# jeffchy/RE2NN-SEQ

Hardware: AMD Instinct MI355X
Metric: tagged tokens/sec @ batch=256, seqlen=64; achieved HBM GB/s vs peak (higher is better)
Workload: dtype f32; 1 GPU; ATIS-BIO-sized onehot i-FST (--method onehot --independent 2): V=950 S=71 C=128, batch 256 x seqlen 64 per GPU, lengths U[5,64]; batches_rotated=4, parallelism=batch-sharded x1 (weights replicated)

## Files before the change

### re2nn-seq_amd/csrc/chain_regs.hip.h

```cpp
#pragma once
#include "common.hip.h"
#include "score_params.hip.h"
#include "launch_order.hip.h"
#include "chain_regs_params.hip.h"
#include "beside.hip.h"

#ifndef FARNN_ABLATE
#define FARNN_ABLATE 0
#endif

namespace farnn {

__device__ __forceinline__ void lds_flag_set(int *f, int v) {
    asm volatile("" ::: "memory");
    __hip_atomic_store(f, v, __ATOMIC_RELAXED, __HIP_MEMORY_SCOPE_WORKGROUP);
}
__device__ __forceinline__ int lds_flag_get(const int *f) {
    const int v = __hip_atomic_load(f, __ATOMIC_RELAXED, __HIP_MEMORY_SCOPE_WORKGROUP);
    asm volatile("" ::: "memory");
    return v;
}
template <int PSTR = RG_PART_STRIDE>
__device__ __forceinline__ int regs_flag_newest(const float *fbase, int lane) {
    const int *f = reinterpret_cast<const int *>(fbase) + 4 * (lane < RG_NWC ? lane : 0);
    const int v0 = lds_flag_get(f), v1 = lds_flag_get(f + PSTR);
    return max(v0, v1);
}
template <int PSTR = RG_PART_STRIDE>
__device__ __forceinline__ bool regs_rows_reached(const float *fbase, int lane, int rows) {
    return __ballot(regs_flag_newest<PSTR>(fbase, lane) < rows + 1) == 0ull;
}
template <int PSTR = RG_PART_STRIDE>
__device__ __forceinline__ int regs_rows_done(const float *fbase, int lane) {
    int v = regs_flag_newest<PSTR>(fbase, lane);
#pragma unroll
    for (int off = 1; off < 8; off <<= 1) v = min(v, __shfl_xor(v, off, WAVE));
    return __builtin_amdgcn_readfirstlane(v) - 1;
}

__device__ __forceinline__ float quad_sum(float x) {
    x += __int_as_float(__builtin_amdgcn_update_dpp(0, __float_as_int(x), 0xB1, 0xf, 0xf, true));
    x += __int_as_float(__builtin_amdgcn_update_dpp(0, __float_as_int(x), 0x4E, 0xf, 0xf, true));
    return x;
}
__device__ __forceinline__ float quad_max(float x) {
    x = fmaxf(x, __int_as_float(__builtin_amdgcn_update_dpp(0, __float_as_int(x), 0xB1, 0xf, 0xf, true)));
    x = fmaxf(x, __int_as_float(__builtin_amdgcn_update_dpp(0, __float_as_int(x), 0x4E, 0xf, 0xf, true)));
    return x;
}

}
#include "chain_wide.hip.h"
#include "chain_dest.hip.h"
namespace farnn {

#if defined(FARNN_PROBES)
constexpr int WG_STAMP_MAX = 4096;
__device__ long long g_wg_stamps[16 * WG_STAMP_MAX];
#define FARNN_RG_STAMP(i) do { if (probe && lane == 0) stamps[i] = (long long)__builtin_amdgcn_s_memtime(); } while (0)
#else
#define FARNN_RG_STAMP(i) do { } while (0)
#endif

template <bool MAXSR, bool SCORE, bool NLX, int RQ = RG_RQ, int D = RG_D, bool LMO = false, bool DEST = false>
__device__ __forceinline__ void chain_regs_body(const RegsParams &p, float *smem, const int tid, const int item, int *b_out) {
    constexpr bool WIDE = RQ != RG_RQ;
    static_assert(!DEST || (!WIDE && !MAXSR), "the destination-split form exists for the narrow kernel and the sum semiring");
    constexpr int PSTR = WIDE ? rgw_part_stride(RQ) : RG_PART_STRIDE;
    constexpr int NG = WIDE ? RGW_NG : RG_NG;
    const int lane = tid & 63;
    const int w = __builtin_amdgcn_readfirstlane(tid >> 6);
    constexpr int nthreads = RG_WAVES * 64;
    const int dir = item & 1, slot = item >> 1;
    const int S = p.S, SP = p.SP, G = p.G, RPG = p.RPG, NP = RG_NWC * G;
    const int PS = WIDE ? p.PS : SP;
    const bool lm_path = SCORE && (LMO || bs_label_map_path(p.sp));
    const RegsLds lds = regs_lds(p.L, SP, NP, p.sp.c16, p.sp.Kc, SCORE, RQ, lm_path, DEST);
    long long *tokoff = reinterpret_cast<long long *>(smem + lds.tok);
    float *part = smem + lds.part, *ol = smem + lds.ol, *hist = smem + lds.hist;
    float *ab = smem + lds.ab, *scl = smem + lds.scl, *obuf = smem + lds.obuf;
    int *misc = reinterpret_cast<int *>(smem + lds.misc);

    int b = p.order ? p.order[slot] : slot;
    int len_sel = -1;
    if (p.sort) b = select_by_length_rank(p.len, p.B, p.L, p.pair ? folded_rank(slot, p.B) : slot, reinterpret_cast<int *>(hist), tid, nthreads, &len_sel);
    if (b_out) *b_out = b;
    const int len = len_sel >= 0 ? len_sel : clamp_len(p.len[b], p.L);
    const int nsteps = p.full ? p.L : len;
    const float *hinit = dir == 0 ? p.h0 : p.hT;
#if defined(FARNN_PROBES)
    __shared__ long long stamps[8];
    const bool quiet = (p.dbg & 2048) != 0;
    const bool probe = ((p.dbg & 32768) && nsteps == p.L && p.L >= 32) || quiet;
    if (w == 0) FARNN_RG_STAMP(0);
#endif

    constexpr bool PRIME_EARLY = DEST && (!SCORE || LMO);
    DestRing<RD_D, RD_LPR> dring;
    if constexpr (PRIME_EARLY)
        if (w < RG_NWC && nsteps > 0) regs_dest_prime<RD_D, RD_LPR>(p, dir, w, lane, nsteps, len, b, dring);
    for (int k = tid; k < nsteps; k += nthreads) {
        const int idx = (dir == 0) ? k : (k < len ? len - 1 - k : k);
        tokoff[k] = (long long)clamp_tok(p.x[(long long)b * p.L + idx], p.V) * p.blk * 4;
    }
    for (int j = tid; j < SP; j += nthreads) ol[j] = (p.o && j < S) ? p.o[j] : 1.0f;
    for (int j = tid; j < (nsteps + 1) * SP; j += nthreads) hist[j] = (j < S) ? hinit[j] : 0.0f;
    if (tid < 32) misc[tid] = tid == RGM_ACQ ? -1 : 0;
    if (tid < 2) part[tid * PSTR + PSTR - 1] = MAXSR ? -INFINITY : 0.0f;
    if (tid < 2 * 4 * RG_NWC) {
        const int fb = tid / (4 * RG_NWC), fk = tid % (4 * RG_NWC);
        part[fb * PSTR + NP * PS + fk] = (DEST && fb == 0 && (fk & 3) == 0) ? __int_as_float(1) : 0.0f;
    }
    if constexpr (DEST) {
        for (int j = tid; j < 2 * RD_XS; j += nthreads)
            smem[lds.xd + j] = j < S ? hinit[j] * ((dir == 1 && p.o) ? p.o[j] : 1.0f) : 0.0f;
    }
    if (WIDE && tid < RG_NWC * RGW_XCH) smem[lds.xch + tid] = 0.0f;
    __syncthreads();
    if (w == 0) FARNN_RG_STAMP(1);
#if FARNN_ABLATE & 256
    return;
#endif

    const float *sflag = part + NP * PS;
    float *stash = (dir == 0 ? p.A : p.Bk) + (long long)b * (p.L + 1) * SP;
    const int ntl = (nsteps + RG_TT - 1) / RG_TT;
    int kmid = 0, pubmax = 0;
    if (SCORE) bs_halves(dir, len, nsteps, kmid, pubmax);
    BesideParams bs;
    bs.A = p.A; bs.Bk = p.Bk; bs.B = p.B; bs.L = p.L; bs.SP = p.SP; bs.CPR = p.CPR; bs.prog = p.prog; bs.arr = p.arr;
    bs.done = p.done; bs.spin = p.spin; bs.dbg = p.dbg; bs.sp = p.sp;
    bs.epoch = (SCORE && w >= RG_NWC) ? (p.done ? bs_launch_epoch(p.done, lane) : p.epoch_host) : 0u;
    int wr_next = 0;
    unsigned lm_pk0 = 0u, lm_pk1 = 0u;
    if (lm_path) lm_load_packed(bs.sp.lm, lane, lm_pk0, lm_pk1);
    if (w < RG_NWC) {
        if constexpr (WIDE) {
            if (nsteps > 0) {
                __builtin_amdgcn_s_setprio(2);
                regs_compute_wide<MAXSR, NLX, RQ, D>(p, dir, w, lane, nsteps, tokoff, part, ol, hist, smem + lds.xch);
                __builtin_amdgcn_s_setprio(0);
                if (w == 0) FARNN_RG_STAMP(2);
#if defined(FARNN_PROBES)
                if (!SCORE && probe && !quiet && w == 0 && lane == 0)
                    printf("seq %d dir %d (wide): setup %lld, chain %lld (%lld per step)\n", b, dir, stamps[1] - stamps[0], stamps[2] - stamps[1],
                           (stamps[2] - stamps[1]) / nsteps);
#endif
            }
        } else if constexpr (DEST) {
            if (nsteps > 0) {
                __builtin_amdgcn_s_setprio(2);
#if defined(FARNN_PROBES)
                const bool probe_ = probe;
#else
                const bool probe_ = false;
#endif
                if constexpr (!PRIME_EARLY) regs_dest_prime<RD_D, RD_LPR>(p, dir, w, lane, nsteps, len, b, dring);
                regs_compute_dest<NLX, RD_D, RD_LPR>(p, dir, w, lane, nsteps, tokoff, part + NP * PS, ol, hist, smem + lds.xd, probe_, b, dring);
                __builtin_amdgcn_s_setprio(0);
                if (w == 0) FARNN_RG_STAMP(2);
#if defined(FARNN_PROBES)
                if (!SCORE && probe && !quiet && w == 0 && lane == 0)
                    printf("seq %d dir %d (destination split): setup %lld, chain %lld (%lld per step)\n", b, dir, stamps[1] - stamps[0], stamps[2] - stamps[1],
                           (stamps[2] - stamps[1]) / nsteps);
#endif
            }
        } else if (nsteps > 0) {
            __builtin_amdgcn_s_setprio(2);
            int g = lane / p.CPR;
            const int c = lane - g * p.CPR;
            const bool active = g < G;
            if (!active) g = 0;
            const int gid = w * G + g, row0 = gid * RPG;
            unsigned voff[RG_RQ];
#pragma unroll
            for (int u = 0; u < RG_RQ; u++) voff[u] = ((unsigned)(row0 + u) * (unsigned)SP + (unsigned)c * 4u) * 4u;
            const char *Mbase = reinterpret_cast<const char *>(dir == 0 ? p.Mf : p.Mb);
            const int rows_w = G * RPG;
            const int rj = lane >> 2, rs = lane & 3;
            const int my_row = w * rows_w + rj;
            const bool my_valid = rj < rows_w && my_row < S;
            const bool my_writer = my_valid && rs == 0;
            const float my_o = my_valid ? ol[my_row] : 1.0f;
            const float c_pre = dir == 0 ? my_o : 1.0f, c_post = dir == 0 ? 1.0f : my_o;
            const float ninf = -INFINITY;
            bool okrow[RG_RQ];
#pragma unroll
            for (int u = 0; u < RG_RQ; u++) okrow[u] = u < RPG && row0 + u < S;
            constexpr int NQI = (RG_NWC * RG_MAXG + 3) / 4;
            const float *ident = part + RG_PART_STRIDE - 1;
            float *dump = part + 2 * RG_PART_STRIDE;
            const float *qptr[NQI];
#pragma unroll
            for (int i = 0; i < NQI; i++)
                qptr[i] = (my_valid && rs + 4 * i < NP) ? part + (rs + 4 * i) * SP + my_row : ident;
            const int nact = G * p.CPR;
            const bool has_flane = nact < 64;
            const bool is_flane = lane == nact;
            float *fslot = part + NP * SP + 4 * w;
            float *wptr = active ? part + gid * SP + c * 4 : (is_flane ? fslot : part + NP * SP + 4 * RG_NWC + (lane - nact) * 4);
// ... 202 lines not shown
            if (SCORE && nsteps > 0 && wr_next > pubmax && done >= nsteps) break;
            const int hi = min(done, (SCORE && wr_next <= pubmax) ? pubmax : nsteps);
            copy_rows(wr_next, hi);
            wr_next = hi + 1;
            if (SCORE && hi < nsteps && published < pubmax) {
                published = hi;
                asm volatile("s_waitcnt vmcnt(0)" ::: "memory");
                if (lane == 0)
                    __hip_atomic_store(p.prog + (long long)dir * p.B + b, ((unsigned long long)bs.epoch << 32) | (unsigned)published,
                                       __ATOMIC_RELAXED, __HIP_MEMORY_SCOPE_AGENT);
            }
        }
    } else if (SCORE) {
        const int fo = bs_flat_offset(bs, b, lane);
        if (lane == 0) misc[RGM_FOFF] = fo;
        const long long foff = fo;
        unsigned mine = 0u;
        int acq = -1;
        const unsigned long long *oprog = p.prog + (long long)(dir ^ 1) * p.B + b;
        const int kfirst = dir == 0 ? kmid : kmid - 1, kstep = dir == 0 ? 1 : -1, klast = dir == 0 ? ntl : -1;
        if constexpr (!LMO)
        for (int k = kfirst; k != klast && !lm_path; k += kstep) {
            int na, nb;
            bs_tile_need(k, len, nsteps, na, nb);
            const int need_own = dir == 0 ? na : nb, need_oth = dir == 0 ? nb : na;
            if (nsteps - need_own < p.solo_margin) break;
            while (!regs_rows_reached<PSTR>(sflag, lane, need_own)) __builtin_amdgcn_s_sleep(4);
            if (need_oth > acq) {
                int pr = -1;
                for (;;) {
                    pr = lane == 0 ? bs_read_prog(oprog, bs.epoch) : 0;
                    pr = __builtin_amdgcn_readfirstlane(pr);
                    if (pr >= need_oth) break;
                    if (regs_rows_reached<PSTR>(sflag, lane, nsteps)) break;
                    __builtin_amdgcn_s_sleep(8);
                }
                if (pr < need_oth) break;
                __builtin_amdgcn_fence(__ATOMIC_ACQUIRE, "agent");
                acq = pr;
            }
            {
                const rg_f32x4 none[NG] = {};
                bs_score_tiles<false, RG_WAVES, NG, RG_NWC>(bs, b, dir, len, nsteps, k, -1, hist, nullptr, nullptr, ab, scl, foff, 0, lane, none);
            }
            mine |= 1u << k;
        }
        {
            int slot = 0;
            for (int k = kfirst; k != klast && slot < RG_NOB; k += kstep) {
                if ((mine >> k) & 1u) continue;
                int na, nb;
                bs_tile_need(k, len, nsteps, na, nb);
                const int need_oth = dir == 0 ? nb : na;
                if (need_oth > acq) {
                    int pr = -1;
                    for (;;) {
                        pr = lane == 0 ? bs_read_prog(oprog, bs.epoch) : 0;
                        pr = __builtin_amdgcn_readfirstlane(pr);
                        if (pr >= need_oth) break;
                        if (regs_rows_reached<PSTR>(sflag, lane, nsteps)) break;
                        __builtin_amdgcn_s_sleep(16);
                    }
                    if (pr < need_oth) break;
                    __builtin_amdgcn_fence(__ATOMIC_ACQUIRE, "agent");
                    acq = pr;
                }
                bs_park_rows<NG, (LMO && WIDE) ? NG / 2 : NG>(bs, b, dir, len, nsteps, k, obuf + slot * RG_TT * SP, lane);
                if (lane == 0) misc[RGM_PARK + slot] = k + 1;
                slot++;
            }
        }
        if (lane == 0) { misc[RGM_MINE] = (int)mine; misc[RGM_ACQ] = acq; }
        FARNN_RG_STAMP(3);
    }
    if constexpr (!SCORE) {
        if (b_out && dir == 0 && w == RG_WAVES - 1) {
            int partsum = 0;
            if (p.sp.flat && !p.sp.offs)
                for (int j = lane; j < b; j += WAVE) partsum += clamp_len(p.len[j], p.L);
#pragma unroll
            for (int off = 32; off >= 1; off >>= 1) partsum += __shfl_xor(partsum, off, WAVE);
            if (lane == 0) { misc[RGM_FOFF] = partsum; misc[RGM_FOFF + 1] = len; }
        }
        return;
    }

    if (w == 0) FARNN_RG_STAMP(4);
    bs_finish<RG_WAVES, NG, RG_WAVES - 1, RG_NWC, true, LMO>(bs, b, dir, len, nsteps, kmid, hist, ab, scl, obuf, misc, w, lane, lm_pk0, lm_pk1, bs.epoch,
        [&]() {
            if (w == RG_NWC)
                for (; wr_next <= nsteps; wr_next++)
                    for (int j = 2 * lane; j < SP; j += 2 * WAVE)
                        st2_agent(stash + (long long)wr_next * SP + j, hist[wr_next * SP + j], hist[wr_next * SP + j + 1]);
        },
        [&]() {
            if (w == RG_NWC) {
                asm volatile("s_waitcnt vmcnt(0)" ::: "memory");
                if (lane == 0)
                    __hip_atomic_store(p.prog + (long long)dir * p.B + b, ((unsigned long long)bs.epoch << 32) | (unsigned)nsteps,
                                       __ATOMIC_RELAXED, __HIP_MEMORY_SCOPE_AGENT);
            }
        });
#if defined(FARNN_PROBES)
    if (quiet && tid == 0 && item < WG_STAMP_MAX) {
        long long *o = g_wg_stamps + 16 * (long long)item + 8;
        o[0] = stamps[1] - stamps[0]; o[1] = stamps[2] - stamps[1]; o[2] = stamps[3] - stamps[2]; o[3] = stamps[4] - stamps[2];
        o[4] = (long long)__builtin_amdgcn_s_memtime() - stamps[4];
    }
    if (probe && !quiet && tid == 0) {
        const long long e = (long long)__builtin_amdgcn_s_memtime();
        printf("seq %d dir %d: setup %lld, chain %lld (%lld per step), scorer alone until +%lld, all waves at the meeting point +%lld, "
               "tiles + arrival %lld; tiles alone %d of %d\n", b, dir, stamps[1] - stamps[0], stamps[2] - stamps[1],
               (stamps[2] - stamps[1]) / nsteps, stamps[3] - stamps[2], stamps[4] - stamps[2], e - stamps[4],
               __popc((unsigned)misc[RGM_MINE]), ntl);
    }
#endif
}

template <bool MAXSR, bool SCORE, bool NLX, bool LMO = false, bool DEST = false>
__global__ void __launch_bounds__(RG_WAVES * 64, 4)
chain_regs_kernel(const RegsParams p) {
    extern __shared__ __align__(16) float smem[];
#if defined(FARNN_PROBES)
    long long w0r = 0, w0c = 0;
    if ((p.dbg & 2048) && threadIdx.x == 0) { w0r = (long long)__builtin_amdgcn_s_memrealtime(); w0c = (long long)__builtin_amdgcn_s_memtime(); }
    int b_probe = -1;
    chain_regs_body<MAXSR, SCORE, NLX, RG_RQ, RG_D, LMO, DEST>(p, smem, (int)threadIdx.x, (int)blockIdx.x, &b_probe);
    if ((p.dbg & 2048) && threadIdx.x == 0 && blockIdx.x < WG_STAMP_MAX) {
        const long long w1r = (long long)__builtin_amdgcn_s_memrealtime(), w1c = (long long)__builtin_amdgcn_s_memtime();
        unsigned hwid, xcc;
        asm volatile("s_getreg_b32 %0, hwreg(HW_REG_HW_ID)" : "=s"(hwid));
        asm volatile("s_getreg_b32 %0, hwreg(HW_REG_XCC_ID)" : "=s"(xcc));
        long long *o = g_wg_stamps + 16 * (long long)blockIdx.x;
        o[0] = b_probe; o[1] = b_probe >= 0 ? (long long)p.len[b_probe] : -1; o[2] = w0r; o[3] = w1r; o[4] = w1c - w0c;
        o[5] = xcc & 15u; o[6] = (hwid >> 13) & 7u; o[7] = (hwid >> 8) & 15u;
    }
#else
    chain_regs_body<MAXSR, SCORE, NLX, RG_RQ, RG_D, LMO, DEST>(p, smem, (int)threadIdx.x, (int)blockIdx.x, nullptr);
#endif
}

template <bool MAXSR, bool SCORE, bool NLX, int RQ, int D>
__global__ void __launch_bounds__(RG_WAVES * 64, 2)
chain_wide_kernel(const RegsParams p) {
    extern __shared__ __align__(16) float smem[];
    chain_regs_body<MAXSR, SCORE, NLX, RQ, D>(p, smem, (int)threadIdx.x, (int)blockIdx.x, nullptr);
}

template <bool MAXSR, bool NLX, int RQ>
__global__ void __launch_bounds__(RG_WAVES * 64, 4)
chain_wide_paired_kernel(const RegsParams p) {
    extern __shared__ __align__(16) float smem[];
    chain_regs_body<MAXSR, true, NLX, RQ, 2, true>(p, smem, (int)threadIdx.x, (int)blockIdx.x, nullptr);
}

}
```

### re2nn-seq_amd/csrc/farnn_hip.hip

```cpp
#include <hip/hip_runtime.h>
#include <hip/hip_ext.h>
#include <stdlib.h>
#include <algorithm>
#include <map>
#include <new>
#include <utility>
#include <vector>

#include "common.hip.h"
#include "host_util.hip.h"
#include "chain.hip.h"
#include "score_decode.hip.h"
#include "layout.hip.h"
#include "fst4_score.hip.h"
#include "decomp_chain.hip.h"
#include "decomp1_score.hip.h"
#include "decomp_rows.hip.h"
#include "compact_tag.hip.h"
#include "decomp_regs.hip.h"
#include "compact.hip.h"
#include "host_util.hip.h"
#include "chain_regs_params.hip.h"

namespace farnn {
// ... 804 lines not shown
        const int lthreads = staged ? 1024 : 256;
        const size_t llds = decomp1_label_lds_bytes(NC, m->RO, m->K, m->Kc, staged, lthreads / 64);
        const int lgrid = std::min((staged ? 1 : 4) * m->n_cu, (B * p.L + lthreads / 64 - 1) / (lthreads / 64));
        if (staged) {
            if ((rc = raise_lds_limit(decomp1_label_kernel<true>, llds))) return rc;
            decomp1_label_kernel<true><<<dim3(lgrid), dim3(lthreads), llds, s>>>(p, m->d1_br, NC, qm.MT, full ? nullptr : m->offs);
        } else {
            decomp1_label_kernel<false><<<dim3(lgrid), dim3(lthreads), llds, s>>>(p, m->d1_br, NC, qm.MT, full ? nullptr : m->offs);
        }
    } else {
        const size_t lds = decomp1_score_lds_bytes(m->S, m->SP, m->Rp, m->ROp, m->Kc);
        if ((rc = raise_lds_limit(decomp1_score_kernel, lds))) return rc;
        decomp1_score_kernel<<<dim3(p.L, B), dim3(256), lds, s>>>(p);
    }
    FARNN_HIP_TRY(hipGetLastError());
    if (m->use_crf) {
        ScoreParams v;
        memset(&v, 0, sizeof(v));
        v.trT = m->tr; v.len = len; v.offs = flat ? m->offs : nullptr; v.tags = tags; v.flat = flat;
        v.crf_scores = m->crf_scores; v.B = B; v.L = m->curL; v.K = m->K; v.Kp = m->Kp;
        v.full = full; v.use_crf = 1; v.o_idx = m->o_idx; v.threshold = m->threshold;
        if ((rc = launch_viterbi(m, v, B, s))) return rc;
    }
    return FARNN_OK;
}

static int launch_decomp0_score(farnn_model *m, const int64_t *x, const int64_t *len, int B, int full,
                                int32_t *tags, int64_t *flat, float *scores, hipStream_t s) {
    Decomp0ScoreParams p;
    p.A = m->A; p.Bk = m->Bk; p.Vgen = m->d0_Vgen; p.S1 = m->dw.S1; p.S2 = m->dw.S2; p.CT = m->d0_CT;
    p.S1w = m->d0_S1w; p.S2w = m->d0_S2w; p.CwT = m->d0_CwT; p.P = m->P;
    p.x = x; p.len = len; p.offs = flat ? m->offs : nullptr;
    p.tags = tags; p.flat = flat; p.scores = scores; p.crf_scores = m->crf_scores;
    p.B = B; p.L = m->curL; p.S = m->S; p.SP = m->SP; p.R = m->R; p.Rp = m->Rp; p.RW = m->RW; p.RWp = m->RWp;
    p.V = m->V;
    p.K = m->K; p.Kp = m->Kp; p.Kc = m->Kc;
    p.full = full; p.use_crf = m->use_crf; p.o_idx = m->o_idx; p.threshold = m->threshold;
    const size_t lds = decomp0_score_lds_bytes(m->SP, m->Rp, m->RWp, m->Kc);
    int rc;
    if ((rc = raise_lds_limit(decomp0_score_kernel, lds))) return rc;
    KernelTimer kt(m, KERN_SCORE, s);
    decomp0_score_kernel<<<dim3((p.L + D0_TOK - 1) / D0_TOK, B), dim3(256), lds, s>>>(p);
    FARNN_HIP_TRY(hipGetLastError());
    if (m->use_crf) {
        ScoreParams v;
        memset(&v, 0, sizeof(v));
        v.trT = m->tr; v.len = len; v.offs = flat ? m->offs : nullptr; v.tags = tags; v.flat = flat;
        v.crf_scores = m->crf_scores; v.B = B; v.L = m->curL; v.K = m->K; v.Kp = m->Kp;
        v.full = full; v.use_crf = 1; v.o_idx = m->o_idx; v.threshold = m->threshold;
        if ((rc = launch_viterbi(m, v, B, s))) return rc;
    }
    return FARNN_OK;
}

static ScoreParams make_score_params(farnn_model *m, const int64_t *len, int B, int full, int32_t *tags,
                                     int64_t *flat, float *scores) {
    ScoreParams p;
    memset(&p, 0, sizeof(p));
    p.A = m->A; p.Bk = m->Bk; p.OT = m->OT; p.OTm = m->OTm; p.c16 = m->c16; p.P = m->P; p.trT = m->tr; p.len = len;
    p.offs = (flat && !m->prep_in_kernel) ? m->offs : nullptr; p.tags = tags; p.flat = flat; p.scores = scores;
    p.crf_scores = m->crf_scores;
    p.B = B; p.L = m->curL; p.S = m->S; p.SP = m->SP; p.K = m->K; p.Kp = m->Kp; p.Kc = m->Kc;
    p.kch = m->Kc / 64;
    p.full = full; p.use_crf = m->use_crf; p.o_idx = m->o_idx; p.threshold = m->threshold;
    p.dbg = tun(TUN_DBG);
    p.kz = (m->kind == KIND_IFST && m->use_crf && !tun(TUN_NOKZ)) ? m->C : 0;
    p.lm = m->lm;
    return p;
}

static int launch_chain_and_decode(farnn_model *m, const int64_t *x, const int64_t *len, int B, int L, int full,
                                   int32_t *tags, int64_t *flat, float *scores, hipStream_t s);

static int launch_score_decode(farnn_model *m, const int64_t *len, int B, int full, int32_t *tags,
                               int64_t *flat, float *scores, hipStream_t s) {
    ScoreParams p = make_score_params(m, len, B, full, tags, flat, scores);
    if (viterbi_can_fuse(m, p)) {
        KernelTimer kt(m, KERN_SCORE, s);
        return launch_viterbi(m, p, B, s, true);
    }
    int rc;
    if (p.lm.on && !p.P && !scores && !m->use_crf && m->S <= LM_MAXS * 2 && (B <= 1024 || !flat || p.offs)) {
        KernelTimer kt(m, KERN_SCORE, s);
        label_map_score_kernel<<<B, LMS_WAVES * 64, 0, s>>>(p);
        FARNN_HIP_TRY(hipGetLastError());
        m->last_lm_score = true;
        return FARNN_OK;
    }
    m->last_lm_score = false;
    const size_t lds = score_lds_bytes(m->S, m->Kc);
    const dim3 grid((p.L + SCORE_TT - 1) / SCORE_TT, B), block(SCORE_WAVES * 64);
    KernelTimer kt(m, KERN_SCORE, s);
#define FARNN_LAUNCH_SCORE(KCH_)                                                              \
    do {                                                                                      \
        if ((rc = raise_lds_limit(score_tile_kernel<KCH_>, lds))) return rc;                  \
        score_tile_kernel<KCH_><<<grid, block, lds, s>>>(p);                                  \
    } while (0)
    switch (p.kch) {
        case 1: FARNN_LAUNCH_SCORE(1); break;
        case 2: FARNN_LAUNCH_SCORE(2); break;
        case 3: FARNN_LAUNCH_SCORE(3); break;
        default: FARNN_LAUNCH_SCORE(4); break;
    }
#undef FARNN_LAUNCH_SCORE
    FARNN_HIP_TRY(hipGetLastError());
    if (m->use_crf && (rc = launch_viterbi(m, p, B, s))) return rc;
    return FARNN_OK;
}

static int launch_chain_and_decode(farnn_model *m, const int64_t *x, const int64_t *len, int B, int L, int full,
                                   int32_t *tags, int64_t *flat, float *scores, hipStream_t s) {
    int rc;
    if (!m->use_crf) {
        const ScoreParams sp = make_score_params(m, len, B, full, tags, flat, scores);
        bool fused = false;
        if ((rc = launch_chain(m, x, len, B, L, full, s, &sp, &fused))) return rc;
        m->last_fused = fused;
        if (fused) return FARNN_OK;
    } else {
        m->last_fused = false;
        const ScoreParams sp = make_score_params(m, len, B, full, tags, flat, scores);
#if defined(FARNN_AB)
        if (tun(TUN_CV_ONE) && m->rgeom.ok && !tun(TUN_NOREGS) && !tun(TUN_NOFUSE) && viterbi_can_fuse(m, sp) &&
            (B <= 1024 || !flat || sp.offs) && chain_viterbi_fits(m->curL, m->SP, m->rgeom.NP, m->K, m->Kp, m->lm.on != 0, m->rgeom.RQ)) {
            const RegsParams rp = make_regs_params(m, x, len, B, full);
            KernelTimer kt(m, KERN_CHAIN, s, true);
            if ((rc = launch_chain_viterbi(rp, sp, m->semiring == FARNN_SEMIRING_MAX, s, kt.e0, kt.e1))) return rc;
            m->last_regs = true; m->last_fused = true;
            return FARNN_OK;
        }
#endif
        if ((rc = launch_chain(m, x, len, B, L, full, s))) return rc;
    }
    return launch_score_decode(m, len, B, full, tags, flat, scores, s);
}

__global__ void clamp_oo_column_kernel(float *scores, long long rows, int K, int col, float threshold) {
    const long long r = (long long)blockIdx.x * blockDim.x + threadIdx.x;
    if (r < rows) {
        const float x = scores[r * K + col];
        scores[r * K + col] = (x < threshold || x != x) ? x : threshold;
    }
}

static int tag_impl(farnn_model *m, const int64_t *x, const int64_t *lengths, int32_t B, int32_t L,
                    int32_t mode, int32_t *tags, int64_t *flat_tags, float *scores, void *stream);

extern "C" int farnn_tag(farnn_model *m, const int64_t *x, const int64_t *lengths, int32_t B, int32_t L,
                         int32_t mode, int32_t *tags, int64_t *flat_tags, float *scores, void *stream) {
    if (!m || !x || !lengths) return fail(FARNN_EINVAL, "tag: null model / x / lengths%s%s");
    if (B <= 0 || L <= 0) return fail(FARNN_EINVAL, "tag: B and L must be positive%s%s");
    if (mode != FARNN_MODE_LOCAL && mode != FARNN_MODE_FULL && mode != FARNN_MODE_RE)
        return fail(FARNN_EINVAL, "tag: bad mode%s%s");
    if (mode != FARNN_MODE_RE) return tag_impl(m, x, lengths, B, L, mode, tags, flat_tags, scores, stream);
    if (m->kind != KIND_IFST && m->kind != KIND_FST4 && m->kind != KIND_IND1)
        return fail(FARNN_EINVAL, "tag: FARNN_MODE_RE exists on the onehot models only (model_onehot.py:148)%s%s");
    int rc = tag_impl(m, x, lengths, B, L, FARNN_MODE_FULL, tags, flat_tags, scores, stream);
    if (rc || !scores) return rc;
    const long long rows = (long long)B * L;
    clamp_oo_column_kernel<<<(unsigned)((rows + 255) / 256), 256, 0, reinterpret_cast<hipStream_t>(stream)>>>(
        scores, rows, m->K, m->C - 1, m->threshold);
    FARNN_HIP_TRY(hipGetLastError());
    return FARNN_OK;
}

static int tag_impl(farnn_model *m, const int64_t *x, const int64_t *lengths, int32_t B, int32_t L,
                    int32_t mode, int32_t *tags, int64_t *flat_tags, float *scores, void *stream) {
// ... 885 lines not shown
    (void)hipDeviceSynchronize();
    for (auto &h : m->hslot) {
        host_slot_free(h);
        if (h.ev_out) (void)hipEventDestroy(h.ev_out);
    }
    if (m->hs_run) (void)hipStreamDestroy(m->hs_run);
    prof_fold(m);
    for (hipEvent_t e : m->prof.pool) (void)hipEventDestroy(e);
    for (void *p : m->owned) (void)hipFree(p);
    if (m->A) (void)hipFree(m->A);
    if (m->Bk) (void)hipFree(m->Bk);
    if (m->offs) (void)hipFree(m->offs);
    if (m->order) (void)hipFree(m->order);
    if (m->crf_scores) (void)hipFree(m->crf_scores);
    if (m->d1_br) (void)hipFree(m->d1_br);
    if (m->hs) (void)hipFree(m->hs);
    if (m->ev_order) (void)hipEventDestroy(m->ev_order);
    delete m;
}

extern "C" int farnn_abi_version(void) { return FARNN_ABI_VERSION; }
extern "C" int farnn_ab_build(void) {
#if defined(FARNN_AB)
    return 1;
#else
    return 0;
#endif
}

extern "C" int farnn_device_count(void) {
    int n = 0;
    if (hipGetDeviceCount(&n) != hipSuccess) return 0;
    return n;
}

extern "C" const char *farnn_last_error(void) { return g_err; }

extern "C" int farnn_num_columns(const farnn_model *m) { return m ? m->K : 0; }

extern "C" double farnn_algorithmic_bytes(const farnn_model *m, int64_t valid_tokens) {
    if (!m) return 0.0;
    const double S = m->S, C = m->C, R = m->R, K = m->K;
    double per_tok = 0.0, once = 0.0;
    switch (m->kind) {
        case KIND_IFST: per_tok = 2.0 * S * S * 4 + 12; break;
        case KIND_IND1: per_tok = 3.0 * S * S * 4 + 12; once = C * S * S * 4; break;
        case KIND_FST4: per_tok = (C + 2.0) * S * S * 4 + 12; break;
        case KIND_DECOMP0:
        case KIND_DECOMP1:
        case KIND_DECOMP:
            per_tok = R * 4 + 12;
            once = (2.0 * S * R + S * S + K * S) * 4;
            break;
    }
    return per_tok * (double)valid_tokens + once;
}

extern "C" double farnn_kernel_algorithmic_bytes(const farnn_model *m, int32_t which, int64_t valid_tokens) {
    if (!m) return 0.0;
    const double S = m->S, C = m->C, R = m->R, K = m->K, n = (double)valid_tokens;
    if (which == KERN_CHAIN) {
        if (m->compact_on) return (2.0 * S * m->bmNS * 8 + 8) * n;
        if (!m->dense_decomp && (m->kind == KIND_DECOMP || m->kind == KIND_DECOMP1 || m->kind == KIND_DECOMP0))
            return (R * 4 + 8) * n + (2.0 * S * R + S * S) * 4;
        return (2.0 * S * S * 4 + 8 + (m->last_fused ? 4 : 0)) * n + (m->last_fused ? K * S * 4 : 0);
    }
    if (which == KERN_SCORE) {
        switch (m->kind) {
            case KIND_FST4: return (C * S * S * 4 + 4) * n;
            case KIND_IND1: return (S * S * 4 + 4) * n + C * S * S * 4;
            default: return 4 * n + K * S * 4;
        }
    }
    return 0.0;
}


#if defined(FARNN_PROBES)
extern "C" int farnn_debug_ct_stamps(long long *out, int n_workgroups) {
    if (!out || n_workgroups < 0 || n_workgroups > farnn::CT_STAMP_MAX) return FARNN_EINVAL;
    if (hipDeviceSynchronize() != hipSuccess) return FARNN_EIO;
    return hipMemcpyFromSymbol(out, HIP_SYMBOL(farnn::g_ct_stamps), sizeof(long long) * 16 * (size_t)n_workgroups) == hipSuccess ? FARNN_OK : FARNN_EIO;
}
#endif
```

### re2nn-seq_amd/csrc/launch_order.hip.h

```cpp
#pragma once
#include "common.hip.h"

namespace farnn {

__device__ __forceinline__ int folded_rank(int slot, int B) {
    const int half = B / 2;
    return slot < half ? slot : (B - 1) - (slot - half);
}

template <int NV>
__device__ __forceinline__ int select_by_length_rank_wave(const int64_t *len, int B, int L, int rank, int lane, int *len_out = nullptr) {
    int v[NV];
#pragma unroll
    for (int i = 0; i < NV; i++) {
        const int k = lane + 64 * i;
        int x = k < B ? (int)len[k] : -1;
        if (k < B) x = x < 0 ? 0 : (x > L ? L : x);
        v[i] = x;
    }
    auto count_ge = [&](int t) {
        int c = 0;
#pragma unroll
        for (int i = 0; i < NV; i++) c += __popcll(__ballot(v[i] >= t));
        return c;
    };
    int lo = 0, hi = L;
    while (lo < hi) {
        const int mid = (lo + hi + 1) >> 1;
        if (count_ge(mid) > rank) lo = mid; else hi = mid - 1;
    }
    const int cls = lo;
    if (len_out) *len_out = cls;
    int rem = rank - count_ge(cls + 1);
    int res = 0;
    bool found = false;
#pragma unroll
    for (int i = 0; i < NV; i++) {
        const unsigned long long m = __ballot(v[i] == cls);
        const int c = __popcll(m);
        if (!found && rem < c) {
            const bool hit = ((m >> lane) & 1ull) && __popcll(m & ((1ull << lane) - 1ull)) == rem;
            res = 64 * i + (int)__builtin_ctzll(__ballot(hit) | (1ull << 63));
            found = true;
        } else if (!found) rem -= c;
    }
    return res;
}

template <bool LDS_ONLY = false>
__device__ __forceinline__ int select_by_length_rank(const int64_t *len, int B, int L, int rank, int *scratch,
                                                     int tid, int , int *len_out = nullptr) {
    if ((tid >> 6) == 0) {
        const int lane = tid & 63;
        int res, cls = 0;
        if (B <= 256) res = select_by_length_rank_wave<4>(len, B, L, rank, lane, &cls);
        else if (B <= 512) res = select_by_length_rank_wave<8>(len, B, L, rank, lane, &cls);
        else res = select_by_length_rank_wave<16>(len, B, L, rank, lane, &cls);
        if (lane == 0) { scratch[0] = res; scratch[1] = cls; }
    }
    if constexpr (LDS_ONLY) wg_barrier_lds(); else __syncthreads();
    const int b = scratch[0], l = scratch[1];
    if constexpr (LDS_ONLY) wg_barrier_lds(); else __syncthreads();
    if (len_out) *len_out = __builtin_amdgcn_readfirstlane(l);
    return __builtin_amdgcn_readfirstlane(b);
}

}
```

### re2nn-seq_amd/csrc/score_decode.hip.h

```cpp
#pragma once
#include <type_traits>
#include "common.hip.h"
#include "score_params.hip.h"
#include "viterbi_hist.hip.h"

namespace farnn {

constexpr int SCORE_KCH = 4;
constexpr int SCORE_WAVES = 8;
constexpr int SCORE_TT = 32;

template <int KCH, bool SC1>
__device__ __forceinline__ void score_tiles(const ScoreParams &p, const int b, const int tile_first, const int tile_step,
                                            float *smem, const int tid, const long long foff_pre = -1, const int len_pre = -1) {
    const int lane = tid & 63;
    const int w = __builtin_amdgcn_readfirstlane(tid >> 6);
    constexpr int nthreads = SCORE_WAVES * 64;
    const int len = len_pre >= 0 ? len_pre : clamp_len(p.len[b], p.L);
    const int nsteps = p.full ? p.L : len;
    const int SP = p.SP, K = p.K, Kc = p.Kc;
    const int ntiles = (p.L + SCORE_TT - 1) / SCORE_TT;

    const int c16 = p.c16;
    const int SPa = 16 * c16 + 4;
// ... 366 lines not shown
        __syncthreads();
        for (int i = tid; i < B; i += 1024) {
            int n = (int)len[i];
            n = n < 0 ? 0 : (n > L ? L : n);
            atomicAdd(&cnt[n], 1);
        }
        __syncthreads();
        {
            const int nb = L + 1, per = (nb + 1023) / 1024;
            const int lo = tid * per, hi = min(lo + per, nb);
            long long s2 = 0;
            for (int r = lo; r < hi; r++) s2 += cnt[L - r];
            __syncthreads();
            sums[tid] = s2;
            __syncthreads();
            for (int off = 1; off < 1024; off <<= 1) {
                long long v = (tid >= off) ? sums[tid - off] : 0;
                __syncthreads();
                sums[tid] += v;
                __syncthreads();
            }
            int run = (tid == 0) ? 0 : (int)sums[tid - 1];
            for (int r = lo; r < hi; r++) { const int c2 = cnt[L - r]; cnt[L - r] = run; run += c2; }
        }
        __syncthreads();
        const int half = B / 2;
        for (int i = tid; i < B; i += 1024) {
            int n = (int)len[i];
            n = n < 0 ? 0 : (n > L ? L : n);
            const int pos = atomicAdd(&cnt[n], 1);
            const int slot = pos < half ? pos : half + (B - 1 - pos);
            order[slot] = i;
        }
    }
}

__global__ void __launch_bounds__(1024)
batch_prep_small_kernel(const int64_t *len, int64_t *offs, int *order, int B, int L, int G) {
    __shared__ __align__(16) int ls[1024];
    const int tid = threadIdx.x;
    for (int k = tid; k < 1024; k += blockDim.x) {
        int v = -1;
        if (k < B) {
            const int n = (int)len[k];
            v = n < 0 ? 0 : (n > L ? L : n);
        }
        ls[k] = v;
    }
    __syncthreads();
    const int i = tid / G, part = tid - i * G;
    const bool live = i < B;
    const int mine = live ? ls[i] : -1;
    int rank = 0;
    unsigned before = 0;
    const int4 *ls4 = reinterpret_cast<const int4 *>(ls);
    const int n4 = (B + 3) >> 2;
    const int per = (n4 + G - 1) / G, lo = part * per, hi = min(lo + per, n4);
#pragma unroll 4
    for (int j4 = lo; j4 < hi; j4++) {
        const int4 v = ls4[j4];
        const int lj[4] = {v.x, v.y, v.z, v.w};
#pragma unroll
        for (int u = 0; u < 4; u++) {
            const int j = j4 * 4 + u;
            rank += (lj[u] > mine) || (lj[u] == mine && j < i);
            before += (j < i && lj[u] > 0) ? (unsigned)lj[u] : 0u;
        }
    }
    for (int off = 1; off < G; off <<= 1) {
        rank += __shfl_xor(rank, off, WAVE);
        before += __shfl_xor(before, off, WAVE);
    }
    if (!live || part != 0) return;
    if (offs) {
        offs[i] = (long long)before;
        if (i == B - 1) offs[B] = (long long)before + mine;
    }
    if (order) {
        const int half = B / 2;
        order[rank < half ? rank : half + (B - 1 - rank)] = i;
    }
}

constexpr int LMS_WAVES = 16;

__global__ void __launch_bounds__(LMS_WAVES * 64)
label_map_score_kernel(const ScoreParams p) {
    const int tid = threadIdx.x, lane = tid & 63;
    const int w = __builtin_amdgcn_readfirstlane(tid >> 6);
    const int b = blockIdx.x;
    const int L = p.L, SP = p.SP;
    const int len = clamp_len(p.len[b], L);
    const int nsteps = p.full ? L : len;
    __shared__ int foff_s;
    if (w == 0) {
        int partsum = 0;
        if (p.flat) {
            if (p.offs) partsum = lane == 0 ? (int)p.offs[b] : 0;
            else for (int j = lane; j < b; j += WAVE) partsum += clamp_len(p.len[j], L);
        }
#pragma unroll
        for (int off = 32; off >= 1; off >>= 1) partsum += __shfl_xor(partsum, off, WAVE);
        if (lane == 0) foff_s = partsum;
    } else if (w == 1 && p.tags) {
        for (int i = nsteps + lane; i < L; i += WAVE) p.tags[(long long)b * L + i] = -1;
    }
    LabelMapRegs lr;
    lm_load(p.lm, lane, lr);
    const bool two = p.lm.nq > 1;
    const float *A = p.A + (long long)b * (L + 1) * SP, *Bk = p.Bk + (long long)b * (L + 1) * SP;
    auto rowB = [&](int i) { return (i + 1 <= len) ? len - (i + 1) : i + 1; };
    float fa0 = 0.f, fa1 = 0.f, ba0 = 0.f, ba1 = 0.f, fb0 = 0.f, fb1 = 0.f, bb0 = 0.f, bb1 = 0.f;
    auto fetch = [&](int q) {
        const int ia = q, ib = q + 1 < nsteps ? q + 1 : q;
        const float *fa = A + (long long)(ia + 1) * SP, *fb = A + (long long)(ib + 1) * SP;
        const float *ba = Bk + (long long)rowB(ia) * SP, *bb = Bk + (long long)rowB(ib) * SP;
        fa0 = fa[lr.st0]; ba0 = ba[lr.st0]; fb0 = fb[lr.st0]; bb0 = bb[lr.st0];
        if (two) { fa1 = fa[lr.st1]; ba1 = ba[lr.st1]; fb1 = fb[lr.st1]; bb1 = bb[lr.st1]; }
    };
    int q = 2 * w;
    if (q < nsteps) fetch(q);
    __syncthreads();
    const long long foff = foff_s;
    for (; q < nsteps; q += 2 * LMS_WAVES) {
        const bool hasb = q + 1 < nsteps;
        const int ia = q, ib = hasb ? q + 1 : q;
        const float xa0 = fa0 * ba0, xa1 = two ? fa1 * ba1 : 0.0f, xb0 = fb0 * bb0, xb1 = two ? fb1 * bb1 : 0.0f;
        if (q + 2 * LMS_WAVES < nsteps) fetch(q + 2 * LMS_WAVES);
        float ya0, ya1, yb0, yb1;
        lm_scan_scores2(lr, xa0, xa1, xb0, xb1, ya0, ya1, yb0, yb1);
        float ma = fmaxf(ya0, ya1), mb = fmaxf(yb0, yb1);
        wave_max_dpp2(ma, mb);
        const int taga = lm_tag_from_candidates(p.lm, lr, ya0, ya1, ma, p.K, p.o_idx);
        const int tagb = lm_tag_from_candidates(p.lm, lr, yb0, yb1, mb, p.K, p.o_idx);
        if (lane < (hasb ? 2 : 1)) {
            const int i = lane ? ib : ia;
            const int tag = lane ? tagb : taga;
            if (p.tags) p.tags[(long long)b * L + i] = tag;
            if (p.flat && i < len) p.flat[foff + i] = tag;
        }
    }
}

}
```

Measured before the change: 302.5 million tokens/s.

## Split label-map scorer into striped workgroups and overlap chain setup with sort

The label-map score kernel now launches several smaller workgroups per sequence, four waves each by default, instead of one sixteen-wave workgroup. Each wave computes its flat offset itself and the LDS barrier is gone, which should give better scheduling and occupancy. In the chain kernel's non-tile forms, wave 0 runs the length-rank selection while the other waves fill the fixed LDS state, and only the padding columns of the history are zeroed. Token offsets are also taken from the dest-prime ring. The cost is repeated prefix-sum work per stripe, and the setup ordering becomes more complex.

```diff
diff --git a/re2nn-seq_amd/csrc/chain_regs.hip.h b/re2nn-seq_amd/csrc/chain_regs.hip.h
--- a/re2nn-seq_amd/csrc/chain_regs.hip.h
+++ b/re2nn-seq_amd/csrc/chain_regs.hip.h
@@ -81,41 +81,88 @@
     float *ab = smem + lds.ab, *scl = smem + lds.scl, *obuf = smem + lds.obuf;
     int *misc = reinterpret_cast<int *>(smem + lds.misc);
 
+    const float *hinit = dir == 0 ? p.h0 : p.hT;
+#if defined(FARNN_PROBES)
+    __shared__ long long stamps[8];
+    if (w == 0 && lane == 0) stamps[0] = stamps[5] = stamps[6] = (long long)__builtin_amdgcn_s_memtime();
+#endif
+    auto fill_fixed = [&](const int t, const int nt) {
+        for (int j = t; j < SP; j += nt) {
+            ol[j] = (p.o && j < S) ? p.o[j] : 1.0f;
+            hist[j] = (j < S) ? hinit[j] : 0.0f;
+        }
+        if (SP > S) {
+            const int npad = SP - S;
+            for (int j = t; j < p.L * npad; j += nt) { const int r = j / npad; hist[(r + 1) * SP + S + (j - r * npad)] = 0.0f; }
+        }
+        if (t < 32) misc[t] = t == RGM_ACQ ? -1 : 0;
+        if (t < 2) part[t * PSTR + PSTR - 1] = MAXSR ? -INFINITY : 0.0f;
+        if (t < 2 * 4 * RG_NWC) {
+            const int fb = t / (4 * RG_NWC), fk = t % (4 * RG_NWC);
+            part[fb * PSTR + NP * PS + fk] = (DEST && fb == 0 && (fk & 3) == 0) ? __int_as_float(1) : 0.0f;
+        }
+        if constexpr (DEST) {
+            for (int j = t; j < 2 * RD_XS; j += nt)
+                smem[lds.xd + j] = j < S ? hinit[j] * ((dir == 1 && p.o) ? p.o[j] : 1.0f) : 0.0f;
+        }
+        if (WIDE && t < RG_NWC * RGW_XCH) smem[lds.xch + t] = 0.0f;
+    };
     int b = p.order ? p.order[slot] : slot;
     int len_sel = -1;
-    if (p.sort) b = select_by_length_rank(p.len, p.B, p.L, p.pair ? folded_rank(slot, p.B) : slot, reinterpret_cast<int *>(hist), tid, nthreads, &len_sel);
+    constexpr bool TILE_FORM = SCORE && !LMO;
+    if (p.sort) {
+        const int rank = p.pair ? folded_rank(slot, p.B) : slot;
+        if constexpr (TILE_FORM) {
+            b = select_by_length_rank(p.len, p.B, p.L, rank, reinterpret_cast<int *>(hist), tid, nthreads, &len_sel);
+        } else {
+            int *sel = reinterpret_cast<int *>(hist + (p.L + 1) * SP);
+            if (w == 0) {
+                const int res = select_by_length_rank_any(p.len, p.B, p.L, rank, lane, &len_sel);
+                if (lane == 0) { sel[0] = res; sel[1] = len_sel; }
+            } else fill_fixed(tid - 64, nthreads - 64);
+            wg_barrier_lds();
+            b = sel[0];
+            len_sel = sel[1];
+        }
+    } else if constexpr (!TILE_FORM) fill_fixed(tid, nthreads);
+    b = __builtin_amdgcn_readfirstlane(b);
+    len_sel = __builtin_amdgcn_readfirstlane(len_sel);
     if (b_out) *b_out = b;
     const int len = len_sel >= 0 ? len_sel : clamp_len(p.len[b], p.L);
     const int nsteps = p.full ? p.L : len;
-    const float *hinit = dir == 0 ? p.h0 : p.hT;
-#if defined(FARNN_PROBES)
-    __shared__ long long stamps[8];
+#if defined(FARNN_PROBES)
     const bool quiet = (p.dbg & 2048) != 0;
     const bool probe = ((p.dbg & 32768) && nsteps == p.L && p.L >= 32) || quiet;
-    if (w == 0) FARNN_RG_STAMP(0);
+    if (w == 0) FARNN_RG_STAMP(5);
 #endif
 
     constexpr bool PRIME_EARLY = DEST && (!SCORE || LMO);
     DestRing<RD_D, RD_LPR> dring;
     if constexpr (PRIME_EARLY)
-        if (w < RG_NWC && nsteps > 0) regs_dest_prime<RD_D, RD_LPR>(p, dir, w, lane, nsteps, len, b, dring);
-    for (int k = tid; k < nsteps; k += nthreads) {
+        if (w < RG_NWC && nsteps > 0) {
+            regs_dest_prime<RD_D, RD_LPR>(p, dir, w, lane, nsteps, len, b, dring);
+            if (w == 0 && lane < nsteps) tokoff[lane] = ((long long)(unsigned)dring.tkw_hi << 32) | (unsigned)dring.tkw_lo;
+        }
+    for (int k = tid + ((PRIME_EARLY && nsteps > 0) ? 64 : 0); k < nsteps; k += nthreads) {
         const int idx = (dir == 0) ? k : (k < len ? len - 1 - k : k);
         tokoff[k] = (long long)clamp_tok(p.x[(long long)b * p.L + idx], p.V) * p.blk * 4;
     }
-    for (int j = tid; j < SP; j += nthreads) ol[j] = (p.o && j < S) ? p.o[j] : 1.0f;
-    for (int j = tid; j < (nsteps + 1) * SP; j += nthreads) hist[j] = (j < S) ? hinit[j] : 0.0f;
-    if (tid < 32) misc[tid] = tid == RGM_ACQ ? -1 : 0;
-    if (tid < 2) part[tid * PSTR + PSTR - 1] = MAXSR ? -INFINITY : 0.0f;
-    if (tid < 2 * 4 * RG_NWC) {
-        const int fb = tid / (4 * RG_NWC), fk = tid % (4 * RG_NWC);
-        part[fb * PSTR + NP * PS + fk] = (DEST && fb == 0 && (fk & 3) == 0) ? __int_as_float(1) : 0.0f;
+    if constexpr (TILE_FORM) {
+        for (int j = tid; j < SP; j += nthreads) ol[j] = (p.o && j < S) ? p.o[j] : 1.0f;
+        for (int j = tid; j < (nsteps + 1) * SP; j += nthreads) hist[j] = (j < S) ? hinit[j] : 0.0f;
+        if (tid < 32) misc[tid] = tid == RGM_ACQ ? -1 : 0;
+        if (tid < 2) part[tid * PSTR + PSTR - 1] = MAXSR ? -INFINITY : 0.0f;
+        if (tid < 2 * 4 * RG_NWC) {
+            const int fb = tid / (4 * RG_NWC), fk = tid % (4 * RG_NWC);
+            part[fb * PSTR + NP * PS + fk] = (DEST && fb == 0 && (fk & 3) == 0) ? __int_as_float(1) : 0.0f;
+        }
+        if constexpr (DEST) {
+            for (int j = tid; j < 2 * RD_XS; j += nthreads)
+                smem[lds.xd + j] = j < S ? hinit[j] * ((dir == 1 && p.o) ? p.o[j] : 1.0f) : 0.0f;
+        }
+        if (WIDE && tid < RG_NWC * RGW_XCH) smem[lds.xch + tid] = 0.0f;
     }
-    if constexpr (DEST) {
-        for (int j = tid; j < 2 * RD_XS; j += nthreads)
-            smem[lds.xd + j] = j < S ? hinit[j] * ((dir == 1 && p.o) ? p.o[j] : 1.0f) : 0.0f;
-    }
-    if (WIDE && tid < RG_NWC * RGW_XCH) smem[lds.xch + tid] = 0.0f;
+    if (w == 0) FARNN_RG_STAMP(6);
     __syncthreads();
     if (w == 0) FARNN_RG_STAMP(1);
 #if FARNN_ABLATE & 256
@@ -484,10 +531,18 @@
             for (int off = 32; off >= 1; off >>= 1) partsum += __shfl_xor(partsum, off, WAVE);
             if (lane == 0) { misc[RGM_FOFF] = partsum; misc[RGM_FOFF + 1] = len; }
         }
+#if defined(FARNN_PROBES)
+        if (quiet && tid == 0 && item < WG_STAMP_MAX && nsteps > 0) {
+            long long *o = g_wg_stamps + 16 * (long long)item + 8;
+            o[0] = stamps[1] - stamps[0]; o[1] = stamps[2] - stamps[1]; o[2] = o[3] = o[4] = 0;
+            o[5] = stamps[5] - stamps[0]; o[6] = stamps[6] - stamps[0];
+        }
+#endif
         return;
     }
 
     if (w == 0) FARNN_RG_STAMP(4);
+    if constexpr (DEST) asm volatile("s_waitcnt vmcnt(0)" ::: "memory");
     bs_finish<RG_WAVES, NG, RG_WAVES - 1, RG_NWC, true, LMO>(bs, b, dir, len, nsteps, kmid, hist, ab, scl, obuf, misc, w, lane, lm_pk0, lm_pk1, bs.epoch,
         [&]() {
             if (w == RG_NWC)
@@ -508,6 +563,7 @@
         long long *o = g_wg_stamps + 16 * (long long)item + 8;
         o[0] = stamps[1] - stamps[0]; o[1] = stamps[2] - stamps[1]; o[2] = stamps[3] - stamps[2]; o[3] = stamps[4] - stamps[2];
         o[4] = (long long)__builtin_amdgcn_s_memtime() - stamps[4];
+        o[5] = stamps[5] - stamps[0]; o[6] = stamps[6] - stamps[0];
     }
     if (probe && !quiet && tid == 0) {
         const long long e = (long long)__builtin_amdgcn_s_memtime();
diff --git a/re2nn-seq_amd/csrc/farnn_hip.hip b/re2nn-seq_amd/csrc/farnn_hip.hip
--- a/re2nn-seq_amd/csrc/farnn_hip.hip
+++ b/re2nn-seq_amd/csrc/farnn_hip.hip
@@ -910,7 +910,7 @@
     int rc;
     if (p.lm.on && !p.P && !scores && !m->use_crf && m->S <= LM_MAXS * 2 && (B <= 1024 || !flat || p.offs)) {
         KernelTimer kt(m, KERN_SCORE, s);
-        label_map_score_kernel<<<B, LMS_WAVES * 64, 0, s>>>(p);
+        label_map_score_kernel<<<B * LMS_STRIPES, LMS_WAVES * 64, 0, s>>>(p);
         FARNN_HIP_TRY(hipGetLastError());
         m->last_lm_score = true;
         return FARNN_OK;
@@ -1962,4 +1962,9 @@
     if (hipDeviceSynchronize() != hipSuccess) return FARNN_EIO;
     return hipMemcpyFromSymbol(out, HIP_SYMBOL(farnn::g_ct_stamps), sizeof(long long) * 16 * (size_t)n_workgroups) == hipSuccess ? FARNN_OK : FARNN_EIO;
 }
+extern "C" int farnn_debug_lms_stamps(long long *out, int n_workgroups) {
+    if (!out || n_workgroups < 0 || n_workgroups > farnn::LMS_STAMP_MAX) return FARNN_EINVAL;
+    if (hipDeviceSynchronize() != hipSuccess) return FARNN_EIO;
+    return hipMemcpyFromSymbol(out, HIP_SYMBOL(farnn::g_lms_stamps), sizeof(long long) * 4 * (size_t)n_workgroups) == hipSuccess ? FARNN_OK : FARNN_EIO;
+}
 #endif
diff --git a/re2nn-seq_amd/csrc/launch_order.hip.h b/re2nn-seq_amd/csrc/launch_order.hip.h
--- a/re2nn-seq_amd/csrc/launch_order.hip.h
+++ b/re2nn-seq_amd/csrc/launch_order.hip.h
@@ -47,15 +47,21 @@
     return res;
 }
 
+__device__ __forceinline__ int select_by_length_rank_any(const int64_t *len, int B, int L, int rank, int lane, int *len_out) {
+    int res;
+    if (B <= 256) res = select_by_length_rank_wave<4>(len, B, L, rank, lane, len_out);
+    else if (B <= 512) res = select_by_length_rank_wave<8>(len, B, L, rank, lane, len_out);
+    else res = select_by_length_rank_wave<16>(len, B, L, rank, lane, len_out);
+    return __builtin_amdgcn_readfirstlane(res);
+}
+
 template <bool LDS_ONLY = false>
 __device__ __forceinline__ int select_by_length_rank(const int64_t *len, int B, int L, int rank, int *scratch,
                                                      int tid, int , int *len_out = nullptr) {
     if ((tid >> 6) == 0) {
         const int lane = tid & 63;
-        int res, cls = 0;
-        if (B <= 256) res = select_by_length_rank_wave<4>(len, B, L, rank, lane, &cls);
-        else if (B <= 512) res = select_by_length_rank_wave<8>(len, B, L, rank, lane, &cls);
-        else res = select_by_length_rank_wave<16>(len, B, L, rank, lane, &cls);
+        int cls = 0;
+        const int res = select_by_length_rank_any(len, B, L, rank, lane, &cls);
         if (lane == 0) { scratch[0] = res; scratch[1] = cls; }
     }
     if constexpr (LDS_ONLY) wg_barrier_lds(); else __syncthreads();
diff --git a/re2nn-seq_amd/csrc/score_decode.hip.h b/re2nn-seq_amd/csrc/score_decode.hip.h
--- a/re2nn-seq_amd/csrc/score_decode.hip.h
+++ b/re2nn-seq_amd/csrc/score_decode.hip.h
@@ -472,32 +472,47 @@
     }
 }
 
-constexpr int LMS_WAVES = 16;
+constexpr int LMS_PER_SEQ = 16;
+#ifndef FARNN_LMS_WAVES
+#define FARNN_LMS_WAVES 4
+#endif
+constexpr int LMS_WAVES = FARNN_LMS_WAVES;
+constexpr int LMS_STRIPES = LMS_PER_SEQ / LMS_WAVES;
+static_assert(LMS_WAVES * LMS_STRIPES == LMS_PER_SEQ, "the stripes of a sequence add up to its sixteen wavefronts");
+
+#if defined(FARNN_PROBES)
+constexpr int LMS_STAMP_MAX = 4096;
+__device__ long long g_lms_stamps[4 * LMS_STAMP_MAX];
+#endif
 
 __global__ void __launch_bounds__(LMS_WAVES * 64)
 label_map_score_kernel(const ScoreParams p) {
     const int tid = threadIdx.x, lane = tid & 63;
-    const int w = __builtin_amdgcn_readfirstlane(tid >> 6);
-    const int b = blockIdx.x;
+    const int b = (int)blockIdx.x / LMS_STRIPES;
+    const int g = ((int)blockIdx.x % LMS_STRIPES) * LMS_WAVES + __builtin_amdgcn_readfirstlane(tid >> 6);
     const int L = p.L, SP = p.SP;
+#if defined(FARNN_PROBES)
+    const bool stamp = (p.dbg & 2048) && tid == 0 && blockIdx.x < LMS_STAMP_MAX;
+    long long *so = g_lms_stamps + 4 * (long long)blockIdx.x;
+    if (stamp) { so[0] = (long long)__builtin_amdgcn_s_memrealtime(); so[1] = so[2] = 0; so[3] = b; }
+#endif
+    unsigned pk0, pk1;
+    lm_load_packed(p.lm, lane, pk0, pk1);
     const int len = clamp_len(p.len[b], L);
+    long long foff = 0;
+    if (p.flat) {
+        if (p.offs) foff = p.offs[b];
+        else {
+            int partsum = 0;
+            for (int j = lane; j < b; j += WAVE) partsum += clamp_len(p.len[j], L);
+#pragma unroll
+            for (int off = 32; off >= 1; off >>= 1) partsum += __shfl_xor(partsum, off, WAVE);
+            foff = partsum;
+        }
+    }
     const int nsteps = p.full ? L : len;
-    __shared__ int foff_s;
-    if (w == 0) {
-        int partsum = 0;
-        if (p.flat) {
-            if (p.offs) partsum = lane == 0 ? (int)p.offs[b] : 0;
-            else for (int j = lane; j < b; j += WAVE) partsum += clamp_len(p.len[j], L);
-        }
-#pragma unroll
-        for (int off = 32; off >= 1; off >>= 1) partsum += __shfl_xor(partsum, off, WAVE);
-        if (lane == 0) foff_s = partsum;
-    } else if (w == 1 && p.tags) {
-        for (int i = nsteps + lane; i < L; i += WAVE) p.tags[(long long)b * L + i] = -1;
-    }
-    LabelMapRegs lr;
-    lm_load(p.lm, lane, lr);
     const bool two = p.lm.nq > 1;
+    const int st0 = (int)(pk0 & 0xffu), st1 = (int)(pk1 & 0xffu);
     const float *A = p.A + (long long)b * (L + 1) * SP, *Bk = p.Bk + (long long)b * (L + 1) * SP;
     auto rowB = [&](int i) { return (i + 1 <= len) ? len - (i + 1) : i + 1; };
     float fa0 = 0.f, fa1 = 0.f, ba0 = 0.f, ba1 = 0.f, fb0 = 0.f, fb1 = 0.f, bb0 = 0.f, bb1 = 0.f;
@@ -505,18 +520,27 @@
         const int ia = q, ib = q + 1 < nsteps ? q + 1 : q;
         const float *fa = A + (long long)(ia + 1) * SP, *fb = A + (long long)(ib + 1) * SP;
         const float *ba = Bk + (long long)rowB(ia) * SP, *bb = Bk + (long long)rowB(ib) * SP;
-        fa0 = fa[lr.st0]; ba0 = ba[lr.st0]; fb0 = fb[lr.st0]; bb0 = bb[lr.st0];
-        if (two) { fa1 = fa[lr.st1]; ba1 = ba[lr.st1]; fb1 = fb[lr.st1]; bb1 = bb[lr.st1]; }
+        fa0 = fa[st0]; ba0 = ba[st0]; fb0 = fb[st0]; bb0 = bb[st0];
+        if (two) { fa1 = fa[st1]; ba1 = ba[st1]; fb1 = fb[st1]; bb1 = bb[st1]; }
     };
-    int q = 2 * w;
+    int q = 2 * g;
     if (q < nsteps) fetch(q);
-    __syncthreads();
-    const long long foff = foff_s;
-    for (; q < nsteps; q += 2 * LMS_WAVES) {
+    if (p.tags)
+        for (int i = nsteps + g * WAVE + lane; i < L; i += LMS_PER_SEQ * WAVE) p.tags[(long long)b * L + i] = -1;
+    LabelMapRegs lr;
+    lm_unpack(p.lm, pk0, pk1, lr);
+#if defined(FARNN_PROBES)
+    bool first = true;
+#endif
+    for (; q < nsteps; q += 2 * LMS_PER_SEQ) {
         const bool hasb = q + 1 < nsteps;
         const int ia = q, ib = hasb ? q + 1 : q;
         const float xa0 = fa0 * ba0, xa1 = two ? fa1 * ba1 : 0.0f, xb0 = fb0 * bb0, xb1 = two ? fb1 * bb1 : 0.0f;
-        if (q + 2 * LMS_WAVES < nsteps) fetch(q + 2 * LMS_WAVES);
+#if defined(FARNN_PROBES)
+        if (stamp && first) { asm volatile("" :: "v"(xa0), "v"(xb0)); so[1] = (long long)__builtin_amdgcn_s_memrealtime(); }
+        first = false;
+#endif
+        if (q + 2 * LMS_PER_SEQ < nsteps) fetch(q + 2 * LMS_PER_SEQ);
         float ya0, ya1, yb0, yb1;
         lm_scan_scores2(lr, xa0, xa1, xb0, xb1, ya0, ya1, yb0, yb1);
         float ma = fmaxf(ya0, ya1), mb = fmaxf(yb0, yb1);
@@ -530,6 +554,9 @@
             if (p.flat && i < len) p.flat[foff + i] = tag;
         }
     }
-}
-
-}
+#if defined(FARNN_PROBES)
+    if (stamp) so[2] = (long long)__builtin_amdgcn_s_memrealtime();
+#endif
+}
+
+}
```

After: 316.7 million tokens/s, median of 6. +4.7%, better.
